# dpryan79/MethylDackel

Hardware: AMD Instinct MI355X
Metric: CpG calls/sec, synthetic 1 Mb contig 30x paired-end WGBS BAM, CpG extract (higher is better)
Workload: dtype u8/u32

## Files before the change

### include/mdk_hip.h

```cpp
#ifndef MDK_HIP_H
#define MDK_HIP_H
#include <stdint.h>
#ifdef __cplusplus
extern "C" {
#endif

#define MDK_ERR_HIP      (-1)
#define MDK_ERR_NODEVICE (-2)
#define MDK_ERR_ARG      (-3)
#define MDK_ERR_NOREF    (-4)
#define MDK_ERR_STRAND0  (-5)
#define MDK_ERR_NOMEM    (-6)
#define MDK_ERR_PREP_HOST (-7)

typedef struct md_dev md_dev;

typedef struct {
    int32_t keepCpG, keepCHG, keepCHH;
    int32_t minPhred;
    int32_t minOppositeDepth;
    int32_t bounds[16];
    int32_t absoluteBounds[16];
    int32_t tile;
    int32_t n_slots;
// ... 99 lines not shown
    float ms_pileup;
    uint64_t algo_bytes;
    uint64_t n_sites;
    int32_t tile, n_tiles, lds_bytes;
} md_bench_result;

int  md_dev_count(void);
int  md_dev_warm(int device);
void md_dev_quiesce(void);
void md_dev_reserve_hint(uint64_t device_bytes);
int  md_dev_open(int device, const md_dev_cfg *cfg, md_dev **out);
int  md_dev_reserve_contigs(md_dev *h, int32_t n);
void md_dev_close(md_dev *h);
const char *md_dev_last_error(void);
int  md_dev_tile(const md_dev *h);

int  md_dev_set_reference(md_dev *h, int32_t tid, const char *seq, int64_t len);

typedef struct { int32_t start, end, strand; } md_region;
int  md_dev_set_regions(md_dev *h, int32_t tid, const md_region *runs, int64_t n);

typedef struct { int32_t len; const uint32_t *count; } md_mbias;
int  md_dev_mbias_submit(md_dev *h, int slot, const md_read_batch *b);
int  md_dev_mbias_submit_raw(md_dev *h, int slot, const md_raw_batch *b);
int  md_dev_mbias_read(md_dev *h, md_mbias *out);
int  md_dev_mbias_reset(md_dev *h);
int  md_dev_slot_sync(md_dev *h, int slot);
int  md_dev_mbias_group(md_dev *h, const int *slots, int n);
int  md_dev_mbias_collect(md_dev *h, const int *slots, int n, int *rc);
int  md_dev_mbias_redone(const md_dev *h);
// ... 172 lines not shown
```

### methyldackel_amd/__init__.py

```python
from __future__ import annotations

import ctypes as C
import os
import struct
import subprocess
from pathlib import Path

ROOT = Path(__file__).resolve().parent
REPO = ROOT.parent
BUILD = Path(os.environ["MDK_BUILD_DIR"]) if os.environ.get("MDK_BUILD_DIR") else ROOT / "_build"
LIB_HIP = BUILD / "libmdk_hip.so"
LIB_EXTRACT = BUILD / "libmdk_extract.so"
CLI = BUILD / "MethylDackel"

CHUNK_NOREF, CHUNK_FOREIGN, CHUNK_BED = 1, 2, 4
CHUNK_EMPTY = CHUNK_NOREF | CHUNK_BED
MDK_ERR = {-1: "HIP call failed", -2: "no device", -3: "bad argument", -4: "reference not uploaded",
           -5: "strand 0 read reached a call", -6: "out of memory"}


class MdkError(RuntimeError):
    pass


# ... 116 lines not shown
    tables = any(bool(raw.range[i].h_rec_off) or bool(raw.range[i].d_rec_off) for i in range(raw.n_ranges))
    if not tables:
        return [raw.rec_off[i] for i in range(raw.n_records)]
    for i in range(raw.n_ranges):
        r = raw.range[i]
        if r.d_rec_off:
            raise MdkError("raw_record_offsets: a range lies in device memory")
        if r.h_rec_off:
            out += [r.h_rec_off[k] - r.rec_delta + o for k in range(r.n_records)]
        else:
            out += [raw.rec_off[hidx + k] for k in range(r.n_records)]; hidx += r.n_records
        o += r.bytes
    return out


HIP_SYMBOLS = ["md_dev_count", "md_dev_warm", "md_dev_quiesce", "md_dev_reserve_hint", "md_dev_open", "md_dev_close", "md_dev_last_error", "md_dev_tile", "md_dev_set_reference", "md_dev_set_regions",
               "md_dev_upload", "md_dev_launch", "md_dev_submit", "md_dev_download", "md_dev_sync", "md_dev_bind_output", "md_dev_wait", "md_sites_order",
               "md_dev_bench", "md_dev_bench_rotate", "md_dev_launch_group", "md_dev_group_max", "md_dev_download_group", "md_dev_reserve_contigs", "md_comm_unique_id", "md_comm_open_rank", "md_comm_open_rank_shared", "md_comm_close", "md_comm_world", "md_comm_gather", "md_comm_wait", "md_comm_result_header", "md_comm_result_send", "md_comm_result_recv", "md_dev_pci_bus_id",
               "md_bench_open", "md_bench_run", "md_bench_verify", "md_bench_region_bytes", "md_bench_close", "md_dev_debug_effective", "md_host_alloc", "md_host_free", "md_host_set_pinned", "md_host_profile", "md_dev_profile_text", "md_host_register", "md_host_register_all",
               "md_dev_set_prep", "md_dev_set_mappability", "md_dev_upload_raw", "md_dev_upload_raw_inplace", "md_dev_upload_wait", "md_dev_upload_done", "md_dev_submit_raw", "md_dev_debug_segments", "md_dev_bench_prep", "md_dev_bench_prep_rotate", "md_bench_set_prep",
               "md_dev_mbias_submit", "md_dev_mbias_submit_raw", "md_dev_mbias_read", "md_dev_mbias_reset", "md_dev_slot_sync",
               "md_dev_mbias_group", "md_dev_mbias_collect", "md_dev_mbias_redone", "md_dev_bias_finish", "md_bias_set_count", "md_bias_set_len", "md_bias_set_redone", "md_bias_set_hist", "md_bias_set_copy", "md_bias_set_free",
               "md_dev_perread_submit", "md_dev_perread_download", "md_dev_perread_submit_raw", "md_dev_perread_download_raw", "md_dev_read_raw",
               "md_piece_members_per_round", "md_piece_create", "md_piece_destroy", "md_piece_submit", "md_piece_wait", "md_piece_read", "md_piece_read_records", "md_piece_copy", "md_piece_bench", "md_piece_bench_crc",
               "md_dev_calls_begin", "md_dev_calls_group", "md_dev_calls_finish", "md_calls_set_count", "md_calls_set_copy", "md_calls_set_free", "md_dev_reset",
               "md_dev_reads_begin", "md_dev_reads_slot", "md_dev_reads_collect", "md_dev_reads_host", "md_dev_reads_finish", "md_reads_set_count", "md_reads_set_name_bytes", "md_reads_set_copy", "md_reads_set_free",
               "md_dev_cytosines_begin", "md_dev_cytosines_group", "md_dev_cytosines_finish", "md_cytosines_set_count", "md_cytosines_set_copy", "md_cytosines_set_free",
               "md_text_open", "md_text_measure_calls", "md_text_measure_cytosines", "md_text_measure_reads", "md_text_fill", "md_text_gather_names", "md_text_close", "md_text_merge_measure", "md_text_merge_fill", "md_text_regions", "md_text_unite_measure", "md_text_unite_fill", "md_text_diff", "md_text_dmr_measure", "md_text_dmr_fill",
               "md_text_reference", "md_text_parse_measure", "md_text_parse_fill_calls", "md_text_parse_fill_cytosines", "md_text_parse_error_offset", "md_text_deflate_measure", "md_text_deflate_fill"]
EXTRACT_SYMBOLS = ["extract_main", "mdk_plan_open", "mdk_plan_close", "mdk_plan_dev_cfg", "mdk_plan_ensure_reference",
                   "mdk_plan_next_chunk", "mdk_plan_try_next_chunk", "mdk_plan_emit", "mdk_plan_finish", "mdk_plan_set_shard", "mdk_plan_n_targets", "mdk_plan_target_name",
# ... 17 lines not shown
        print(r.stdout[-4000:], r.stderr[-4000:])
    if r.returncode:
        raise MdkError("build failed")


def lib_hip():
    global _hip
    if _hip is None:
        if not LIB_HIP.exists():
            raise MdkError(f"{LIB_HIP} is missing: the HIP extension was not built (run `make` / __graft_entry__.build()); there is no fallback")
        L = C.CDLL(str(LIB_HIP), mode=C.RTLD_GLOBAL)
        L.md_dev_last_error.restype = C.c_char_p
        L.md_dev_open.argtypes = [C.c_int, C.POINTER(md_dev_cfg), C.POINTER(C.c_void_p)]
        L.md_dev_close.argtypes = [C.c_void_p]
        L.md_dev_tile.argtypes = [C.c_void_p]
        L.md_dev_set_reference.argtypes = [C.c_void_p, C.c_int32, C.c_char_p, C.c_int64]
        L.md_dev_set_regions.argtypes = [C.c_void_p, C.c_int32, C.POINTER(md_region), C.c_int64]
        for f in ("md_dev_upload", "md_dev_submit"):
            getattr(L, f).argtypes = [C.c_void_p, C.c_int, C.POINTER(md_read_batch)]
        L.md_dev_launch.argtypes = [C.c_void_p, C.c_int]
        L.md_dev_download.argtypes = [C.c_void_p, C.c_int, C.POINTER(md_sites)]
        L.md_dev_sync.argtypes = [C.c_void_p]
        L.md_dev_bind_output.argtypes = [C.c_void_p, C.c_int, C.c_void_p, C.c_void_p, C.c_void_p, C.c_int64, C.c_int64]
        L.md_dev_wait.argtypes = [C.c_void_p, C.c_int, C.POINTER(md_sites_dev)]
        L.md_sites_order.argtypes = [C.c_void_p, C.c_void_p, C.c_void_p, C.c_int32, C.c_int64, C.c_void_p, C.c_void_p]
        L.md_sites_order.restype = C.c_int64
        L.md_dev_bench.argtypes = [C.c_void_p, C.c_int, C.c_int, C.c_int, C.POINTER(md_bench_result)]
        L.md_dev_bench_rotate.argtypes = [C.c_void_p, C.POINTER(C.c_int), C.c_int, C.c_int, C.c_int, C.c_int, C.POINTER(md_bench_result)]
        L.md_dev_launch_group.argtypes = [C.c_void_p, C.POINTER(C.c_int), C.c_int]
        L.md_comm_unique_id.argtypes = [C.c_char_p]
# ... 1723 lines not shown
```

### methyldackel_amd/csrc/mdk_hip.hip

```cpp
#include <sys/mman.h>
#include <atomic>
#include <mutex>
#include <algorithm>
#include <type_traits>
#include <condition_variable>
#include <thread>
#include <chrono>
#include "mdk_hip_internal.hpp"

#define DEFAULT_TILE 2048
#define PERMAX 4
#define MAX_TILE (WG * PERMAX)
#define LDS_LIMIT 163840

static thread_local char g_err[MDK_ERR_BYTES] = "";
char *mdk_err_buf() { return g_err; }
int fail(int code, const char *what, hipError_t e) {
    snprintf(g_err, sizeof(g_err), "%s: %s", what, e == hipSuccess ? "invalid argument" : hipGetErrorString(e));
    return code;
}

static std::atomic<uint64_t> g_prof_ns[PF_N], g_prof_calls[PF_N];
bool mdk_prof_on() { static const bool on = getenv("MDK_HOST_PROFILE") != nullptr; return on; }
double mdk_now() { return std::chrono::duration<double>(std::chrono::steady_clock::now().time_since_epoch()).count(); }
// ... 122 lines not shown
    p = harena_take(256); if(p) harena_give(p);
}


struct KParams {
    const md_seg *seg; const uint8_t *blob;
    const uint8_t *ctxcode; int64_t reflen;
    int64_t beg, end; int tile, ntiles, nper;
    const TileEnt *tiles;
    md_site *site; md_site_var *var; md_tile_seg *tseg; uint32_t *total, *total_next; int64_t cap_sites;
    int keepmask, minPhred;
    int bounds[16], abounds[16];
    int *err;
    int packed;
    int mbias; uint32_t *hist; int hist_lq;
};

__device__ __forceinline__ void trim_window(const KParams &P, int strand, int read2, int lq, int &lo, int &hi) {
    if(strand < 1) { lo = 0; hi = lq; return; }
    int b = 4 * (strand - 1) + (read2 ? 2 : 0);
    int lb = P.bounds[b], rb = P.bounds[b + 1];
    int alb = P.abounds[b], arb = P.abounds[b + 1];
    lb = lb < lq ? lb : lq; alb = alb < lq ? alb : lq; arb = arb < lq ? arb : lq;
    lo = lb > alb ? lb : alb;
    hi = (rb && rb < lq) ? rb : lq;
    if(lq - arb < hi) hi = lq - arb;
}

struct RD {
    int lq, lo, hi;
    const uint8_t *seq, *qual;
};
__device__ __forceinline__ RD make_rd(const KParams &P, uint32_t off4, uint32_t lq, int strand, int read2) {
    RD d; d.lq = (int)lq;
    if(P.packed) { d.seq = P.blob + off4; d.qual = d.seq + ((d.lq + 1) >> 1); }
    else { d.seq = P.blob + 4ull * off4; d.qual = d.seq + ((((d.lq + 1) >> 1) + 3) & ~3); }
    trim_window(P, strand, read2, d.lq, d.lo, d.hi);
    return d;
}

#include "mdk_overlap_rule.h"

__global__ __launch_bounds__(WG) void k_classify(const char *ref, uint8_t *code, int64_t n) {
    for(int64_t p = (int64_t)blockIdx.x * WG + threadIdx.x; p < n; p += (int64_t)gridDim.x * WG) {
        char c = ref[p] & 0x5f; int type, isG, out = 0;
        if(c == 'C') {
            isG = 0;
            if(p + 1 < n && (ref[p + 1] & 0x5f) == 'G') type = 0;
            else if(p + 2 < n && (ref[p + 2] & 0x5f) == 'G') type = 1;
            else type = 2;
            out = 1 + 2 * type + isG;
        } else if(c == 'G') {
// ... 10 lines not shown
__global__ __launch_bounds__(WG) void k_mask_regions(uint8_t *code, int64_t n, const md_region *runs, int64_t nruns) {
    for(int64_t p = (int64_t)blockIdx.x * WG + threadIdx.x; p < n; p += (int64_t)gridDim.x * WG) {
        const int c = code[p] & 15;
        if(!c) { code[p] = 0; continue; }
        int64_t a = 0, b = nruns;
        while(a < b) { const int64_t m = (a + b) >> 1; if((int64_t)runs[m].end <= p) a = m + 1; else b = m; }
        code[p] = (a < nruns && (int64_t)runs[a].start <= p) ? (uint8_t)(c | ((runs[a].strand & 3) << 4)) : (uint8_t)0;
    }
}

#define KB 2

template <bool VARIANT>
__device__ __forceinline__ void lane_seg(const KParams &P, const md_seg &g, int T0, int T1,
                                         const uint16_t *listC, int nC, const uint16_t *listG, int nG,
                                         uint32_t *cm, uint32_t *cu, uint32_t *co, uint32_t *cv) {
    const int send = g.rpos + (int)g.len;
    if(g.rpos >= T1 || send <= T0) return;
    const int strand = g.sf & MDK_SF_STRAND;
    const bool odd = strand & 1, second = (g.sf & MDK_SF_SECOND) != 0, partner = (g.sf & MDK_SF_PARTNER) != 0;
    const RD o = make_rd(P, g.off4, g.l_qseq, strand, g.sf & MDK_SF_READ2);
    RD m = o;
    if(partner) m = make_rd(P, g.m_off4, g.m_l_qseq, g.msf & MDK_SF_STRAND, g.msf & MDK_SF_READ2);
    const int lo_off = g.rpos > T0 ? g.rpos - T0 : 0, hi_off = (send < T1 ? send : T1) - T0;
    const int badrs = strand == 0 ? 6 : (odd ? 4 : 2);
#pragma unroll
    for(int pass = 0; pass < (VARIANT ? 2 : 1); pass++) {
        const bool callpass = pass == 0;
        const bool useC = (odd == callpass);
        const uint16_t *list = useC ? listC : listG; const int n = useC ? nC : nG;
        int a = 0, b = n;
        while(a < b) { int mid = (a + b) >> 1; if((int)(list[mid] & 0x1fff) < lo_off) a = mid + 1; else b = mid; }
        int i = a;
        while(i < n) {
            int li[KB];
#pragma unroll
            for(int k = 0; k < KB; k++) {
                li[k] = -1;
                if(i < n) { const int e = list[i], l = e & 0x1fff; if(l < hi_off) { li[k] = ((badrs >> (e >> 13)) & 1) ? -2 : l; i++; } else i = n; }
            }
            if(li[0] == -1) break;
            uint32_t sb[KB], qb[KB], msb[KB], mqb[KB];
#pragma unroll
            for(int k = 0; k < KB; k++) {
                sb[k] = 0xff; qb[k] = 0; msb[k] = 0xff; mqb[k] = 0;
                if(li[k] >= 0) {
                    const int d = T0 + li[k] - g.rpos, q = (int)g.q0 + d, mq = (int)g.m_q0 + d;
                    if(q >= o.lo && q < o.hi) { sb[k] = o.seq[q >> 1]; qb[k] = o.qual[q]; }
                    if(partner && mq >= m.lo && mq < m.hi) { msb[k] = m.seq[mq >> 1]; mqb[k] = m.qual[mq]; }
                }
            }
#pragma unroll
            for(int k = 0; k < KB; k++) {
                if(li[k] < 0) continue;
                const int d = T0 + li[k] - g.rpos, q = (int)g.q0 + d, mq = (int)g.m_q0 + d;
                int bq = (q & 1) ? (sb[k] & 15) : (sb[k] >> 4), ql = (int)qb[k];
                if(partner) { int mb = (mq & 1) ? (msb[k] & 15) : (msb[k] >> 4); ql = resolve_overlap(second, bq, ql, mb, (int)mqb[k]); }
                if(callpass) {
                    if(strand == 0) atomicExch(P.err, 1);
                    if(ql >= P.minPhred) {
                        if(odd) { if(bq == 2) atomicAdd(&cm[li[k]], 1u); else if(bq == 8) atomicAdd(&cu[li[k]], 1u); }
                        else { if(bq == 4) atomicAdd(&cm[li[k]], 1u); else if(bq == 1) atomicAdd(&cu[li[k]], 1u); }
                    }
                } else if(VARIANT) {
                    if(ql >= P.minPhred) {
                        atomicAdd(&co[li[k]], 1u);
// ... 185 lines not shown
    lds_barrier();
    int pre = incl - packed, tot = 0;
    for(int w = 0; w < WAVES; w++) { const int c = wsum[w]; if(w < wave) pre += c; tot += c; }
    nC = tot & 0xffff; nG = tot >> 16;
    int oc = pre & 0xffff, og = pre >> 16;
#pragma unroll
    for(int j = 0; j < PERMAX; j++) {
        if(j < PER && code[j]) {
            const uint16_t ent = (uint16_t)((tid * PER + j) | ((code[j] >> 4) << 13));
            if((code[j] - 1) & 1) listG[og++] = ent; else listC[oc++] = ent;
        }
    }
    lds_barrier();
}

template <bool VARIANT, bool QW>
__device__ __forceinline__ void pileup_tile(const KParams &P, const int t, const int b) {
    extern __shared__ __align__(16) uint32_t lds[];
    const int TILE = P.tile, PER = TILE / WG;
    uint32_t *cm = lds, *cu = lds + TILE, *co = lds + 2 * TILE, *cv = lds + 3 * TILE;
    uint16_t *listC = (uint16_t *)(lds + (VARIANT ? 4 : 2) * TILE), *listG = listC + TILE;
    __shared__ int wsum[WAVES];
    __shared__ uint32_t sbase;

    const int64_t T0 = P.beg + (int64_t)t * TILE;
    const int64_t T1 = (T0 + TILE < P.end) ? T0 + TILE : P.end;
    const int tlen = (int)(T1 - T0);
    const int tid = threadIdx.x, lane = tid & 63, wave = tid >> 6;
    if(t == 0 && tid == 0) *P.total_next = 0;

    const TileEnt te = P.tiles[t];
    const int first = te.last > te.first ? te.first : 0, last = te.last > te.first ? te.last : 0;
    int code[PERMAX];
    load_codes(P, T0, tlen, PER, tid, code);
    md_seg g0; g0.rpos = 0x7fffffff; g0.len = 0;
    if(first + tid < last) g0 = P.seg[first + tid];

#pragma unroll
    for(int j = 0; j < PERMAX; j++) {
        if(j < PER) {
            const int i = tid * PER + j;
            cm[i] = 0; cu[i] = 0;
            if(VARIANT) { co[i] = 0; cv[i] = 0; }
        }
    }
    int nC, nG;
    build_lists(P, PER, tid, lane, wave, code, listC, listG, wsum, nC, nG);

    uint32_t codes = 0;
#pragma unroll
    for(int j = 0; j < PERMAX; j++) codes |= (uint32_t)(code[j] & 0xff) << (8 * j);
    asm volatile("" : "+v"(codes));

    if constexpr(QW) {
        const int topC = nC ? 1 << (31 - __clz(nC)) : 0, topG = nG ? 1 << (31 - __clz(nG)) : 0;
        for(int r0 = first; r0 < last; r0 += WG) {
            md_seg g = g0;
            if(r0 != first) { g.rpos = 0x7fffffff; g.len = 0; if(r0 + tid < last) g = P.seg[r0 + tid]; }
#ifndef QW_NO_SORT
            const SegQ sq = seg_sort(seg_setup<VARIANT>(P, g, (int)T0, (int)T1, listC, nC, nG, topC, topG), lane);
#else
            const SegQ sq = seg_setup<VARIANT>(P, g, (int)T0, (int)T1, listC, nC, nG, topC, topG);
#endif
            quarter_sites<VARIANT>(P, sq, lane, listC, cm, cu, co, cv);
        }
    } else {
        if(first + tid < last) lane_seg<VARIANT>(P, g0, (int)T0, (int)T1, listC, nC, listG, nG, cm, cu, co, cv);
        for(int r = first + WG + tid; r < last; r += WG) {
            const md_seg g = P.seg[r];
            lane_seg<VARIANT>(P, g, (int)T0, (int)T1, listC, nC, listG, nG, cm, cu, co, cv);
        }
    }
    uint32_t reserved = 0;
    if(tid == 0) reserved = (nC + nG) ? atomicAdd(P.total, (uint32_t)(nC + nG)) : 0u;
    __syncthreads();

#pragma unroll
    for(int j = 0; j < PERMAX; j++) code[j] = (int)((codes >> (8 * j)) & 0xffu);
    uint32_t vm[PERMAX], vu[PERMAX], vo[PERMAX], vv[PERMAX]; int cnt = 0;
#pragma unroll
    for(int j = 0; j < PERMAX; j++) {
        vm[j] = vu[j] = vo[j] = vv[j] = 0;
        const int i = tid * PER + j;
        if(j < PER && i < tlen && code[j]) { vm[j] = cm[i]; vu[j] = cu[i]; if(VARIANT) { vo[j] = co[i]; vv[j] = cv[i]; } }
        if((vm[j] + vu[j]) > 0 || vo[j] > 0) cnt++;
    }
    const int incl = wave_scan_incl(cnt, lane);
    if(lane == 63) wsum[wave] = incl;
    if(tid == 0) sbase = reserved;
    __syncthreads();
    if(tid == 0) {
        int tot = 0; for(int w = 0; w < WAVES; w++) tot += wsum[w];
        md_tile_seg sg; sg.off = reserved; sg.cnt = (uint32_t)tot; P.tseg[t] = sg;
    }
    {
        uint32_t o = sbase + (uint32_t)(incl - cnt);
        for(int w = 0; w < wave; w++) o += (uint32_t)wsum[w];
#pragma unroll
        for(int j = 0; j < PERMAX; j++) {
            if((vm[j] + vu[j]) > 0 || vo[j] > 0) {
                if((int64_t)o < P.cap_sites) {
                    md_site rec; rec.pos = (uint32_t)(T0 + tid * PER + j); rec.nmeth = vm[j]; rec.nunmeth = vu[j]; rec.meta = (uint32_t)((code[j] & 15) - 1);
                    P.site[o] = rec;
                    if(VARIANT) { md_site_var rv; rv.noff = vo[j]; rv.nvar = vv[j]; P.var[o] = rv; }
                }
                o++;
            }
        }
// ... 315 lines not shown
    if(side_streams) { std::unique_lock<std::mutex> lk(g_stash_mu); g_stash_cv.wait_for(lk, std::chrono::milliseconds(500), [] { return g_warm_streams_made.load() >= WARM_STREAMS; }); }
    else for(int i = 0; i < WARM_STREAMS; i++) {
        hipStream_t s = nullptr;
        if(hipStreamCreateWithFlags(&s, hipStreamNonBlocking) != hipSuccess) { (void)hipGetLastError(); break; }
        { std::lock_guard<std::mutex> lk(g_stash_mu);
          if(g_stash_dev != device) { g_stash.clear(); g_stash_dev = device; }
          g_stash.push_back(s); }
        g_stash_cv.notify_all();
    }
    const double t4 = mdk_now();
    arena_prime(device);
    if(mdk_prof_on()) fprintf(stderr, "[mdk hip] warm-up: runtime init + device count %.3fs, context (hipSetDevice + hipFree(0)) %.3fs, the library's code object %.3fs, %d streams %.3fs, first blocks of carved device / pinned memory %.3fs\n", t1 - t0, t2 - t1, t3 - t2, WARM_STREAMS, t4 - t3, mdk_now() - t4);
    return 0;
}

static int fixed_lds(int tile, bool variant) { return tile * ((variant ? 16 : 8) + 4); }

extern "C" int md_dev_open(int device, const md_dev_cfg *cfg, md_dev **out) {
    if(!cfg || !out) return fail(MDK_ERR_ARG, "md_dev_open", hipSuccess);
    *out = nullptr;
    const double t_open0 = mdk_now();
    for(int q = 0; q < 256; q++) {
        uint8_t v = (uint8_t)q; v = (uint8_t)(int)(v + 0.2 * v);
        if(v != (uint8_t)(((q * 6) / 5) & 255)) { snprintf(g_err, sizeof(g_err), "boost identity fails at q=%d", q); return MDK_ERR_ARG; }
    }
    int n = md_dev_count();
    if(n <= 0) { if(n == 0) snprintf(g_err, sizeof(g_err), "no HIP device visible"); return MDK_ERR_NODEVICE; }
    if(device < 0 || device >= n) return fail(MDK_ERR_ARG, "md_dev_open: device index", hipSuccess);
    HIPCHK(hipSetDevice(device));
    g_warm_reg_stop.store(true);
    if(code_object_load()) return fail(MDK_ERR_HIP, "loading the device library's code object", hipGetLastError());
    md_dev *h = new md_dev();
    h->device = device; h->cfg = *cfg;
    h->tile = cfg->tile > 0 ? cfg->tile : ((cfg->keepCHG || cfg->keepCHH) ? 1536 : DEFAULT_TILE);
    h->tile = (h->tile + WG - 1) / WG * WG;
    if(h->tile > MAX_TILE) h->tile = MAX_TILE;
    h->n_slots = cfg->n_slots > 0 ? cfg->n_slots : 2;
    h->variant = cfg->minOppositeDepth > 0;
    h->qw = (cfg->keepCHG || cfg->keepCHH) && !getenv("MDK_NO_QW");
    while(fixed_lds(h->tile, h->variant) > LDS_LIMIT - 1024 && h->tile > WG) h->tile -= WG;
    if(fixed_lds(h->tile, h->variant) > 65536) {
        HIPCHK(hipFuncSetAttribute(pileup_fn(h->variant, h->qw), hipFuncAttributeMaxDynamicSharedMemorySize, fixed_lds(h->tile, h->variant)));
        HIPCHK(hipFuncSetAttribute(pileup_multi_fn(h->variant, h->qw), hipFuncAttributeMaxDynamicSharedMemorySize, fixed_lds(h->tile, h->variant)));
    }
    h->slots.resize(h->n_slots);
    if(h->d_status.need((size_t)h->n_slots) || h->h_status.need((size_t)h->n_slots)) return MDK_ERR_NOMEM;
    HIPCHK(hipMemset(h->d_status.p, 0, sizeof(SlotStatus) * (size_t)h->n_slots));
    HIPCHK(hipDeviceSynchronize());
    memset(h->h_status.p, 0, sizeof(SlotStatus) * (size_t)h->n_slots);
    for(int i = 0; i < h->n_slots; i++) { Slot &s = h->slots[i]; s.index = i; s.d_total.p = h->d_status.p[i].total; s.d_err.p = &h->d_status.p[i].err; s.d_pcnt.p = &h->d_status.p[i].pc; s.h_st.p = &h->h_status.p[i]; }
    const double t_open1 = mdk_now();
    const bool shared = cfg->n_streams > 0;
    const int n_streams = shared ? std::min(cfg->n_streams, (h->n_slots + MAXM - 1) / MAXM) : h->n_slots;
    for(int i = 0; i < n_streams; i++) { hipStream_t st = stream_take(device); if(!st) return fail(MDK_ERR_HIP, "hipStreamCreateWithFlags", hipGetLastError()); h->streams.push_back(st); }
    for(auto &s : h->slots) {
        s.stream = h->streams[(size_t)(shared ? s.index / MAXM : s.index) % (size_t)n_streams];
        HIPCHK(hipEventCreate(&s.e0)); HIPCHK(hipEventCreate(&s.e1)); HIPCHK(hipEventCreate(&s.k0)); HIPCHK(hipEventCreate(&s.k1));
        s.run = s.stream;
    }
// ... 62 lines not shown
    for(Slot &s : h->slots) {
        slot_buffers_release(s);
        Slot f;
        f.stream = s.stream; f.e0 = s.e0; f.e1 = s.e1; f.k0 = s.k0; f.k1 = s.k1; f.index = s.index; f.run = s.stream; f.ring = s.ring;
        s = f;
    }
    h->d_status.release(); h->h_status.release();
    mdk_debug_state("md_dev_reset, released");
    arena_restart_if_idle(h->device); harena_restart_if_idle();
    if(h->d_status.need((size_t)h->n_slots) || h->h_status.need((size_t)h->n_slots)) return MDK_ERR_NOMEM;
    HIPCHK(hipMemset(h->d_status.p, 0, sizeof(SlotStatus) * (size_t)h->n_slots));
    HIPCHK(hipDeviceSynchronize());
    memset(h->h_status.p, 0, sizeof(SlotStatus) * (size_t)h->n_slots);
    for(Slot &s : h->slots) { s.d_total.p = h->d_status.p[s.index].total; s.d_err.p = &h->d_status.p[s.index].err; s.d_pcnt.p = &h->d_status.p[s.index].pc; s.h_st.p = &h->h_status.p[s.index]; }
    h->cfg = *cfg;
    h->tile = cfg->tile > 0 ? cfg->tile : ((cfg->keepCHG || cfg->keepCHH) ? 1536 : DEFAULT_TILE);
    h->tile = (h->tile + WG - 1) / WG * WG;
    if(h->tile > MAX_TILE) h->tile = MAX_TILE;
    h->variant = cfg->minOppositeDepth > 0;
    h->qw = (cfg->keepCHG || cfg->keepCHH) && !getenv("MDK_NO_QW");
    while(fixed_lds(h->tile, h->variant) > LDS_LIMIT - 1024 && h->tile > WG) h->tile -= WG;
    if(fixed_lds(h->tile, h->variant) > 65536) {
        HIPCHK(hipFuncSetAttribute(pileup_fn(h->variant, h->qw), hipFuncAttributeMaxDynamicSharedMemorySize, fixed_lds(h->tile, h->variant)));
        HIPCHK(hipFuncSetAttribute(pileup_multi_fn(h->variant, h->qw), hipFuncAttributeMaxDynamicSharedMemorySize, fixed_lds(h->tile, h->variant)));
    }
    return 0;
}

extern "C" int md_dev_tile(const md_dev *h) { return h ? h->tile : MDK_ERR_ARG; }

extern "C" int md_dev_reserve_contigs(md_dev *h, int32_t n) {
    if(!h || n < 0) return fail(MDK_ERR_ARG, "md_dev_reserve_contigs", hipSuccess);
    const size_t k = (size_t)n;
    if(h->ref.size() < k) { h->ref.resize(k, nullptr); h->refcode.resize(k, nullptr); h->reflen.resize(k, 0); }
    if(h->ref_carved.size() < k) h->ref_carved.resize(k, 0);
    if(h->d_runs.size() < k) { h->d_runs.resize(k, nullptr); h->n_runs.resize(k, 0); h->has_runs.resize(k, 0); }
    if(h->mapbits.size() < k) { h->mapbits.resize(k, nullptr); h->maplen.resize(k, 0); }
    return 0;
}

static void ref_release(md_dev *h, size_t tid) {
// ... 76 lines not shown
    if(b->tid < 0 || (size_t)b->tid >= h->ref.size() || !h->ref[b->tid]) { snprintf(g_err, sizeof(g_err), "reference for tid %d not uploaded", b->tid); return MDK_ERR_NOREF; }
    HIPCHK(hipSetDevice(h->device));
    if(s->busy) {
        HIPCHK(hipStreamSynchronize(s->stream));
        if(s->run && s->run != s->stream) HIPCHK(hipStreamSynchronize(s->run));
    }
    s->busy = true;
    s->fresh = true;
    if((uint64_t)b->blob_bytes >= (1ull << 32) - 64) return fail(MDK_ERR_ARG, "md_dev_upload: more than 4 GiB of read payload in one chunk", hipSuccess);
    const int64_t span = b->end - b->beg;
    s->n_segs = b->n_segs; s->n_reads = b->n_reads; s->tid = b->tid; s->beg = b->beg; s->end = b->end; s->uploaded = false; s->launched = false; s->raw_layout = false;
    const int TILE = h->tile;
    const int ntiles = (int)((span + TILE - 1) / TILE);
    if(s->h_tiles.need((size_t)(ntiles > 0 ? ntiles : 1))) return MDK_ERR_NOMEM;
    build_tiles(b, TILE, s->h_tiles.p, ntiles);
    s->tile = TILE; s->ntiles = ntiles; s->lds_bytes = fixed_lds(TILE, h->variant);
    s->read_bytes = b->algo_bytes;
    size_t ns = (size_t)b->n_segs, nt = (size_t)(ntiles > 0 ? ntiles : 1);
    if(s->d_seg_in.need(ns + 1) || s->d_blob.need((size_t)b->blob_bytes + 64)) return MDK_ERR_NOMEM;
    if(s->d_tiles.need(nt) || s->d_seg.need(nt)) return MDK_ERR_NOMEM;
    if(!s->b_site) {
        if(s->d_site.need((size_t)span + 16)) return MDK_ERR_NOMEM;
        if(h->variant && s->d_var.need((size_t)span + 16)) return MDK_ERR_NOMEM;
    }
    if(ns) {
        host_block_ensure_registered(b->seg); host_block_ensure_registered(b->blob);
        HIPCHK(hipMemcpyAsync(s->d_seg_in.p, b->seg, ns * sizeof(md_seg), hipMemcpyHostToDevice, s->stream));
        HIPCHK(hipMemcpyAsync(s->d_blob.p, b->blob, (size_t)b->blob_bytes, hipMemcpyHostToDevice, s->stream));
    }
    if(ntiles) HIPCHK(hipMemcpyAsync(s->d_tiles.p, s->h_tiles.p, nt * sizeof(TileEnt), hipMemcpyHostToDevice, s->stream));
    s->uploaded = true;
// ... 12 lines not shown
static int fill_kparams(md_dev *h, Slot *s, KParams &P) {
    memset(&P, 0, sizeof(P));
    P.seg = s->d_seg_in.p; P.blob = s->raw_layout ? const_cast<uint8_t *>(s->raw_at) : s->d_blob.p; P.packed = s->raw_layout ? 1 : 0;
    P.ctxcode = h->refcode[s->tid]; P.reflen = h->reflen[s->tid];
    P.beg = s->beg; P.end = s->end; P.tile = s->tile; P.ntiles = s->ntiles; P.nper = (s->ntiles + 7) / 8;
    P.tiles = s->d_tiles.p;
    if(s->b_site) {
        if(s->b_cap_tiles < s->ntiles) return fail(MDK_ERR_ARG, "bound tile-segment buffer too small", hipSuccess);
        P.site = s->b_site; P.var = s->b_var; P.tseg = s->b_seg; P.cap_sites = s->b_cap_sites;
    } else { P.site = s->d_site.p; P.var = s->d_var.p; P.tseg = s->d_seg.p; P.cap_sites = (int64_t)s->d_site.cap; }
    P.total = s->d_total.p + (s->ring % RING); P.total_next = s->d_total.p + ((s->ring + 1) % RING);
    P.keepmask = (h->cfg.keepCpG ? 1 : 0) | (h->cfg.keepCHG ? 2 : 0) | (h->cfg.keepCHH ? 4 : 0);
    P.minPhred = h->cfg.minPhred;
    for(int i = 0; i < 16; i++) { P.bounds[i] = h->cfg.bounds[i]; P.abounds[i] = h->cfg.absoluteBounds[i]; }
    P.err = s->d_err.p;
    return 0;
}

int launch_kernels(md_dev *h, Slot *s, bool time_pileup, hipStream_t on) {
    hipStream_t st = on ? on : s->stream;
    if(s->fresh && st != s->stream) { HIPCHK(hipEventRecord(s->e0, s->stream)); HIPCHK(hipStreamWaitEvent(st, s->e0, 0)); }
    if(s->raw_layout && s->prep_pending) { Slot *one[1] = {s}; int rc = enqueue_prep_group(h, one, 1, st); if(rc) return rc; }
    s->fresh = false; s->run = st; s->packed = false;
    s->ring++;
    if(s->ntiles > 0) {
        KParams P; int rc = fill_kparams(h, s, P); if(rc) return rc;
        int grid = P.nper * 8;
        if(time_pileup) HIPCHK(hipEventRecord(s->k0, st));
        launch_pileup(h, grid, (size_t)s->lds_bytes, st, P);
        if(time_pileup) HIPCHK(hipEventRecord(s->k1, st));
// ... 688 lines not shown
```

### methyldackel_amd/csrc/mdk_hip_internal.hpp

```cpp
#ifndef MDK_HIP_INTERNAL_HPP
#define MDK_HIP_INTERNAL_HPP
#include <hip/hip_runtime.h>
#include <stdint.h>
#include <stdio.h>
#include <stdlib.h>
#include <string.h>
#include <atomic>
#include <vector>
#include <mutex>
#include "mdk_hip.h"

#ifndef WG
#define WG 512
#endif
#define WAVES (WG / 64)
#define RING 64
#define MAXM 8

#define MDK_HIDDEN __attribute__((visibility("hidden")))
MDK_HIDDEN char *mdk_err_buf();
#define MDK_ERR_BYTES 512
MDK_HIDDEN int fail(int code, const char *what, hipError_t e);
#define HIPCHK(call) do { hipError_t e_ = (call); if(e_ != hipSuccess) return fail(MDK_ERR_HIP, #call, e_); } while(0)

MDK_HIDDEN int mdk_mark_begin(const char *what);
// ... 73 lines not shown
    int n_segs = 0, n_reads = 0, ntiles = 0, tid = -1, tile = 0, lds_bytes = 0; int64_t beg = 0, end = 0; uint64_t read_bytes = 0;
    bool uploaded = false, launched = false; unsigned ring = 0;
    double t_launch = 0;
    bool packed = false;
    bool busy = false;
};

struct CallsState;
MDK_HIDDEN void calls_state_free(md_dev *h);
struct ReadsState;
MDK_HIDDEN void reads_state_free(md_dev *h);
struct CytoState;
MDK_HIDDEN void cyto_state_free(md_dev *h);
struct md_dev {
    int device; md_dev_cfg cfg; int tile, n_slots; bool variant; bool qw = false;
    CallsState *calls = nullptr; bool no_pack = false;
    ReadsState *reads = nullptr; bool reads_on = false;
    CytoState *cyto = nullptr;
    std::vector<hipStream_t> streams;
    std::mutex crc_mu; void *d_crc = nullptr;
    std::mutex piece_mu; std::vector<hipStream_t> piece_streams; int piece_rr = 0; hipStream_t piece_in = nullptr, piece_inf = nullptr;
    hipStream_t ref_stream = nullptr;
    std::vector<Slot> slots;
    std::vector<char *> ref; std::vector<uint8_t *> refcode; std::vector<int64_t> reflen; std::vector<char> ref_carved; std::vector<int64_t> refcap;
    DBuf<SlotStatus> d_status; HBuf<SlotStatus> h_status;
    md_prep_cfg prep; bool prep_set = false; std::vector<uint32_t *> mapbits; std::vector<int64_t> maplen;
    std::vector<md_region *> d_runs; std::vector<int64_t> n_runs; std::vector<char> has_runs;
    uint32_t *d_hist = nullptr; int hist_cap = 0, hist_len = 0; std::vector<uint32_t> h_hist;
    std::mutex mb_mu; int mb_redone = 0, mb_hint = 0;
    std::atomic<bool> scan_wide{getenv("MDK_SCAN_WIDE") && atoi(getenv("MDK_SCAN_WIDE")) > 0}; bool scan_wide_fixed = getenv("MDK_SCAN_WIDE") != nullptr;
// ... 47 lines not shown
    if(lane == 63) wtot[wave] = x;
    __syncthreads();
    T before = 0; total = 0;
    for(int w = 0; w < WGS / 64; w++) { const T t = wtot[w]; if(w < wave) before += t; total += t; }
    __syncthreads();
    return before + x - v;
}

enum { PF_UP_SYNC = 0, PF_UP_ALLOC, PF_UP_COPY, PF_LAUNCH, PF_FIN_WAIT, PF_DL_COPY, PF_DL_ORDER, PF_SETREF, PF_PIECE_SUBMIT, PF_PIECE_WAIT, PF_GRP_DEV, PF_GRP_TURN, PF_N };
MDK_HIDDEN bool mdk_prof_on();
MDK_HIDDEN void mdk_prof_add(int site, double seconds);
MDK_HIDDEN double mdk_now();
struct ProfScope { int site; double t0; ProfScope(int s) : site(s), t0(mdk_prof_on() ? mdk_now() : 0.0) {} ~ProfScope() { if(mdk_prof_on()) mdk_prof_add(site, mdk_now() - t0); } };
MDK_HIDDEN Slot *get_slot(md_dev *h, int slot);
MDK_HIDDEN void host_block_ensure_registered(const void *ptr);
MDK_HIDDEN int launch_kernels(md_dev *h, Slot *s, bool time_pileup, hipStream_t on = nullptr);
MDK_HIDDEN int launch_group_on(md_dev *h, const int *slots, int n, hipStream_t on, bool cross_sync);
MDK_HIDDEN int64_t finish_count(md_dev *h, Slot *s);
MDK_HIDDEN int64_t finish_eval(md_dev *h, Slot *s);
MDK_HIDDEN int finish_group(md_dev *h, const int *slots, int n, int64_t *counts);
MDK_HIDDEN int prep_outcome(md_dev *h, Slot *s);
MDK_HIDDEN int prep_kernels_init();
MDK_HIDDEN void inflate_kernels_warm();
MDK_HIDDEN hipStream_t mdk_piece_stream_take(int device);
MDK_HIDDEN hipStream_t mdk_stream_take(int device);
MDK_HIDDEN void mdk_debug_state(const char *where);
MDK_HIDDEN int mbias_drain(md_dev *h);
MDK_HIDDEN int enqueue_prep_group(md_dev *h, Slot *const *ss, int n, hipStream_t st);
struct ColSpec { uint32_t elem, extra; };
#define COLTAB_MAXK 8
// ... 52 lines not shown
```

### methyldackel_amd/csrc/mdk_prep.hip

```cpp
#include <algorithm>
#include <atomic>
#include <mutex>
#include "mdk_hip_internal.hpp"
#include "mdk_pair_rule.h"

#ifndef PB
#define PB 256
#endif
#define MAXG 16
#define CNT_READY 0x80000000u

__device__ __forceinline__ uint32_t ld16(const uint8_t *p) { uint16_t v; __builtin_memcpy(&v, p, 2); return v; }
__device__ __forceinline__ uint32_t ld32(const uint8_t *p) { uint32_t v; __builtin_memcpy(&v, p, 4); return v; }
__device__ __forceinline__ uint64_t ld64(const uint8_t *p) { uint64_t v; __builtin_memcpy(&v, p, 8); return v; }
__device__ __forceinline__ uint4 ld128(const uint8_t *p) { uint4 v; __builtin_memcpy(&v, p, 16); return v; }

struct PrepParams {
    const uint8_t *raw; uint64_t raw_bytes; const uint32_t *rec_off; int n_rec;
    md_prep_cfg cfg; int32_t tid; int64_t beg, end, woff, wlen;
    const char *ref; int64_t reflen;
    const uint32_t *mapbits; int64_t maplen;
    const md_region *runs; int64_t nruns; int bed_on;
    PrepRead *rd; uint32_t *aidx;
    unsigned long long *hent; int32_t *hnext, *hfwd; uint32_t hmask;
// ... 1015 lines not shown
        ~SlowCall() { if(on) { const double t = mdk_now(); if(t - t0 > 0.004) { char w[256]; snprintf(w, sizeof(w), "slow upload_raw: %.1f ms (slot wait %.1f, buffers %.1f, copies %.1f), %d ranges, %d records, first range %s", (t - t0) * 1e3, (t_sync - t0) * 1e3, (t_alloc - t_sync) * 1e3, (t - t_alloc) * 1e3, b->n_ranges, b->n_records, b->n_ranges ? (b->range[0].d_rec_off ? "device" : b->range[0].h_rec_off ? "host+table" : "host") : "-"); mdk_marks_dump(w); } } } } slow(b);
    if(s->busy) {
        ProfScope pf(PF_UP_SYNC);
        HIPCHK(hipStreamSynchronize(s->stream));
        if(s->run && s->run != s->stream) HIPCHK(hipStreamSynchronize(s->run));
    }
    slow.t_sync = slow.on ? mdk_now() : 0;
    s->busy = true;
    s->fresh = true;
    uint64_t total = 0;
    for(int i = 0; i < b->n_ranges; i++) total += b->range[i].bytes;
    if(total >= (1ull << 32) - 64) return fail(MDK_ERR_ARG, "md_dev_upload_raw: more than 4 GiB of records in one chunk", hipSuccess);
    const int64_t span = b->end - b->beg; const int TILE = h->tile;
    const int ntiles = (int)((span + TILE - 1) / TILE), n = b->n_records, nb = (n + PB - 1) / PB;
    s->tid = b->tid; s->beg = b->beg; s->end = b->end; s->woff = b->woff; s->wlen = b->wlen; s->uploaded = false; s->launched = false;
    s->tile = TILE; s->ntiles = ntiles; s->lds_bytes = TILE * ((h->variant ? 16 : 8) + 4);
    s->pr_nrec = n; s->raw_bytes = total; s->raw_layout = true; s->n_segs = -1; s->n_reads = -1; s->read_bytes = 0;
    static const bool no_inplace = getenv("MDK_NO_INPLACE") != nullptr;
    const bool inplace = may_stay && !no_inplace && b->n_ranges == 1 && b->range[0].d_rec_off && (uint32_t)n == b->range[0].n_records && n > 0 && b->range[0].bytes + (uint64_t)b->range[0].rec_delta < (1ull << 32) - 64;
    const size_t nn = (size_t)n + 1, nt = (size_t)(ntiles > 0 ? ntiles : 1);
    const size_t segcap = std::max<size_t>(s->d_seg_in.cap, nn * 2 + 4096);
    s->hmask = pow2_at_least(nn + nn / 4) - 1;
    static std::atomic<int> first_call{1}; const bool first = mdk_prof_on() && first_call.exchange(0); const double tf0 = first ? mdk_now() : 0; double tf1 = 0;
    {
        ProfScope pf(PF_UP_ALLOC);
        if((!inplace && (s->d_raw.need((size_t)total + 64) || s->d_recoff.need(nn))) || s->d_prd.need(nn) || s->d_hnext.need(2 * nn + 8) || s->d_zero.need(zero_bytes_for(s->hmask, nb)) ||
           s->d_seg_in.need(segcap) || s->d_tiles.need(nt) || s->d_seg.need(nt)) return MDK_ERR_NOMEM;
        if(!s->b_site) {
            if(s->d_site.need((size_t)span + 16)) return MDK_ERR_NOMEM;
            if(h->variant && s->d_var.need((size_t)span + 16)) return MDK_ERR_NOMEM;
        }
// ... 151 lines not shown
```

Before: 6.866 billion.

## Prefetch pileup segments into LDS with async global_load_lds double buffering

Adds per-wave LDS staging windows, sized to fit in LDS left over without lowering workgroups per CU. Each wave prefetches the next batch of 32-byte segment records into LDS with inline global_load_lds_dwordx4 while it processes the current batch. This hides global latency in the segment loop. The trim bounds move into an LDS table, and the atomic output reservation moves earlier onto a thread in the last wave so it overlaps the segment work. Risks include fragile inline asm with manual m0 and waitcnt handling, and extra LDS per block.

```diff
diff --git a/include/mdk_hip.h b/include/mdk_hip.h
--- a/include/mdk_hip.h
+++ b/include/mdk_hip.h
@@ -137,6 +137,7 @@
 void md_dev_close(md_dev *h);
 const char *md_dev_last_error(void);
 int  md_dev_tile(const md_dev *h);
+int  md_dev_stage_segments(md_dev *h);
 
 int  md_dev_set_reference(md_dev *h, int32_t tid, const char *seq, int64_t len);
 
diff --git a/methyldackel_amd/__init__.py b/methyldackel_amd/__init__.py
--- a/methyldackel_amd/__init__.py
+++ b/methyldackel_amd/__init__.py
@@ -154,7 +154,7 @@
     return out
 
 
-HIP_SYMBOLS = ["md_dev_count", "md_dev_warm", "md_dev_quiesce", "md_dev_reserve_hint", "md_dev_open", "md_dev_close", "md_dev_last_error", "md_dev_tile", "md_dev_set_reference", "md_dev_set_regions",
+HIP_SYMBOLS = ["md_dev_count", "md_dev_warm", "md_dev_quiesce", "md_dev_reserve_hint", "md_dev_open", "md_dev_close", "md_dev_last_error", "md_dev_tile", "md_dev_stage_segments", "md_dev_set_reference", "md_dev_set_regions",
                "md_dev_upload", "md_dev_launch", "md_dev_submit", "md_dev_download", "md_dev_sync", "md_dev_bind_output", "md_dev_wait", "md_sites_order",
                "md_dev_bench", "md_dev_bench_rotate", "md_dev_launch_group", "md_dev_group_max", "md_dev_download_group", "md_dev_reserve_contigs", "md_comm_unique_id", "md_comm_open_rank", "md_comm_open_rank_shared", "md_comm_close", "md_comm_world", "md_comm_gather", "md_comm_wait", "md_comm_result_header", "md_comm_result_send", "md_comm_result_recv", "md_dev_pci_bus_id",
                "md_bench_open", "md_bench_run", "md_bench_verify", "md_bench_region_bytes", "md_bench_close", "md_dev_debug_effective", "md_host_alloc", "md_host_free", "md_host_set_pinned", "md_host_profile", "md_dev_profile_text", "md_host_register", "md_host_register_all",
@@ -202,6 +202,7 @@
         L.md_dev_open.argtypes = [C.c_int, C.POINTER(md_dev_cfg), C.POINTER(C.c_void_p)]
         L.md_dev_close.argtypes = [C.c_void_p]
         L.md_dev_tile.argtypes = [C.c_void_p]
+        L.md_dev_stage_segments.argtypes = [C.c_void_p]
         L.md_dev_set_reference.argtypes = [C.c_void_p, C.c_int32, C.c_char_p, C.c_int64]
         L.md_dev_set_regions.argtypes = [C.c_void_p, C.c_int32, C.POINTER(md_region), C.c_int64]
         for f in ("md_dev_upload", "md_dev_submit"):
diff --git a/methyldackel_amd/csrc/mdk_hip.hip b/methyldackel_amd/csrc/mdk_hip.hip
--- a/methyldackel_amd/csrc/mdk_hip.hip
+++ b/methyldackel_amd/csrc/mdk_hip.hip
@@ -160,13 +160,16 @@
     int *err;
     int packed;
     int mbias; uint32_t *hist; int hist_lq;
+    int stage_waves;
 };
 
-__device__ __forceinline__ void trim_window(const KParams &P, int strand, int read2, int lq, int &lo, int &hi) {
+template <bool TB = false>
+__device__ __forceinline__ void trim_window(const KParams &P, int strand, int read2, int lq, int &lo, int &hi, const int *tb = nullptr) {
     if(strand < 1) { lo = 0; hi = lq; return; }
     int b = 4 * (strand - 1) + (read2 ? 2 : 0);
-    int lb = P.bounds[b], rb = P.bounds[b + 1];
-    int alb = P.abounds[b], arb = P.abounds[b + 1];
+    int lb, rb, alb, arb;
+    if constexpr(TB) { lb = tb[b]; rb = tb[b + 1]; alb = tb[16 + b]; arb = tb[16 + b + 1]; }
+    else { lb = P.bounds[b]; rb = P.bounds[b + 1]; alb = P.abounds[b]; arb = P.abounds[b + 1]; }
     lb = lb < lq ? lb : lq; alb = alb < lq ? alb : lq; arb = arb < lq ? arb : lq;
     lo = lb > alb ? lb : alb;
     hi = (rb && rb < lq) ? rb : lq;
@@ -177,11 +180,12 @@
     int lq, lo, hi;
     const uint8_t *seq, *qual;
 };
-__device__ __forceinline__ RD make_rd(const KParams &P, uint32_t off4, uint32_t lq, int strand, int read2) {
+template <bool TB = false>
+__device__ __forceinline__ RD make_rd(const KParams &P, uint32_t off4, uint32_t lq, int strand, int read2, const int *tb = nullptr) {
     RD d; d.lq = (int)lq;
     if(P.packed) { d.seq = P.blob + off4; d.qual = d.seq + ((d.lq + 1) >> 1); }
     else { d.seq = P.blob + 4ull * off4; d.qual = d.seq + ((((d.lq + 1) >> 1) + 3) & ~3); }
-    trim_window(P, strand, read2, d.lq, d.lo, d.hi);
+    trim_window<TB>(P, strand, read2, d.lq, d.lo, d.hi, tb);
     return d;
 }
 
@@ -222,14 +226,14 @@
 template <bool VARIANT>
 __device__ __forceinline__ void lane_seg(const KParams &P, const md_seg &g, int T0, int T1,
                                          const uint16_t *listC, int nC, const uint16_t *listG, int nG,
-                                         uint32_t *cm, uint32_t *cu, uint32_t *co, uint32_t *cv) {
+                                         uint32_t *cm, uint32_t *cu, uint32_t *co, uint32_t *cv, const int *tb) {
     const int send = g.rpos + (int)g.len;
     if(g.rpos >= T1 || send <= T0) return;
     const int strand = g.sf & MDK_SF_STRAND;
     const bool odd = strand & 1, second = (g.sf & MDK_SF_SECOND) != 0, partner = (g.sf & MDK_SF_PARTNER) != 0;
-    const RD o = make_rd(P, g.off4, g.l_qseq, strand, g.sf & MDK_SF_READ2);
+    const RD o = make_rd<true>(P, g.off4, g.l_qseq, strand, g.sf & MDK_SF_READ2, tb);
     RD m = o;
-    if(partner) m = make_rd(P, g.m_off4, g.m_l_qseq, g.msf & MDK_SF_STRAND, g.msf & MDK_SF_READ2);
+    if(partner) m = make_rd<true>(P, g.m_off4, g.m_l_qseq, g.msf & MDK_SF_STRAND, g.msf & MDK_SF_READ2, tb);
     const int lo_off = g.rpos > T0 ? g.rpos - T0 : 0, hi_off = (send < T1 ? send : T1) - T0;
     const int badrs = strand == 0 ? 6 : (odd ? 4 : 2);
 #pragma unroll
@@ -258,6 +262,8 @@
                     if(partner && mq >= m.lo && mq < m.hi) { msb[k] = m.seq[mq >> 1]; mqb[k] = m.qual[mq]; }
                 }
             }
+#pragma unroll
+            for(int k = 0; k < KB; k++) asm volatile("" :: "v"(sb[k]), "v"(qb[k]), "v"(msb[k]), "v"(mqb[k]));
 #pragma unroll
             for(int k = 0; k < KB; k++) {
                 if(li[k] < 0) continue;
@@ -473,6 +479,20 @@
     lds_barrier();
 }
 
+#define RSV_TID (WG - 64)
+
+__device__ __forceinline__ void stage_segs(const md_seg *seg, const int base, const int last, int tid, const uint32_t win) {
+    asm volatile("" : "+v"(tid));
+#pragma unroll
+    for(int k = 0; k < 2; k++) {
+        const int p = 64 * k + (tid & 63), s = base + (p >> 1);
+        if(s < last) {
+            const uint8_t *src = (const uint8_t *)(seg + s) + 16 * (p & 1); uint32_t keep;
+            asm volatile("s_mov_b32 %0, m0\n\ts_mov_b32 m0, %2\n\ts_nop 0\n\tglobal_load_lds_dwordx4 %1, off\n\ts_mov_b32 m0, %0" : "=&s"(keep) : "v"(src), "s"(__builtin_amdgcn_readfirstlane(win + 1024u * k)) : "memory");
+        }
+    }
+}
+
 template <bool VARIANT, bool QW>
 __device__ __forceinline__ void pileup_tile(const KParams &P, const int t, const int b) {
     extern __shared__ __align__(16) uint32_t lds[];
@@ -481,6 +501,7 @@
     uint16_t *listC = (uint16_t *)(lds + (VARIANT ? 4 : 2) * TILE), *listG = listC + TILE;
     __shared__ int wsum[WAVES];
     __shared__ uint32_t sbase;
+    __shared__ int tbl[32];
 
     const int64_t T0 = P.beg + (int64_t)t * TILE;
     const int64_t T1 = (T0 + TILE < P.end) ? T0 + TILE : P.end;
@@ -494,6 +515,17 @@
     load_codes(P, T0, tlen, PER, tid, code);
     md_seg g0; g0.rpos = 0x7fffffff; g0.len = 0;
     if(first + tid < last) g0 = P.seg[first + tid];
+    const int *const tb = tbl;
+    if(!QW && wave == WAVES - 1) {
+        int v = 0;
+#pragma unroll
+        for(int i = 0; i < 16; i++) { if(lane == i) v = P.bounds[i]; if(lane == 16 + i) v = P.abounds[i]; }
+        if(lane < 32) tbl[lane] = v;
+    }
+    const int uwave = __builtin_amdgcn_readfirstlane(wave);
+    const uint32_t win = (uint32_t)(uintptr_t)(__attribute__((address_space(3))) uint8_t *)((uint8_t *)(listC + 2 * TILE) + MDK_STAGE_WAVE_BYTES * uwave);
+    const bool staged = !QW && uwave < P.stage_waves;
+    if(staged) stage_segs(P.seg, first + WG + 64 * uwave, last, tid, win);
 
 #pragma unroll
     for(int j = 0; j < PERMAX; j++) {
@@ -505,6 +537,8 @@
     }
     int nC, nG;
     build_lists(P, PER, tid, lane, wave, code, listC, listG, wsum, nC, nG);
+
+    if(tid == RSV_TID) sbase = (nC + nG) ? atomicAdd(P.total, (uint32_t)(nC + nG)) : 0u;
 
     uint32_t codes = 0;
 #pragma unroll
@@ -524,14 +558,27 @@
             quarter_sites<VARIANT>(P, sq, lane, listC, cm, cu, co, cv);
         }
     } else {
-        if(first + tid < last) lane_seg<VARIANT>(P, g0, (int)T0, (int)T1, listC, nC, listG, nG, cm, cu, co, cv);
-        for(int r = first + WG + tid; r < last; r += WG) {
-            const md_seg g = P.seg[r];
-            lane_seg<VARIANT>(P, g, (int)T0, (int)T1, listC, nC, listG, nG, cm, cu, co, cv);
-        }
-    }
-    uint32_t reserved = 0;
-    if(tid == 0) reserved = (nC + nG) ? atomicAdd(P.total, (uint32_t)(nC + nG)) : 0u;
+        if(first + tid < last) lane_seg<VARIANT>(P, g0, (int)T0, (int)T1, listC, nC, listG, nG, cm, cu, co, cv, tb);
+        if(staged) {
+            for(int rb = first + WG + 64 * uwave; rb < last; rb += WG) {
+                asm volatile("s_waitcnt vmcnt(0)" ::: "memory");
+                __builtin_amdgcn_wave_barrier();
+                int l = tid; asm volatile("" : "+v"(l)); l &= 63;
+                const uint4 *const rec = (const uint4 *)((__attribute__((address_space(3))) uint8_t *)(uintptr_t)win + 32 * l);
+                uint4 w0 = rec[0], w1 = rec[1];
+                asm volatile("s_waitcnt lgkmcnt(0)" : "+v"(w0.x), "+v"(w0.y), "+v"(w0.z), "+v"(w0.w), "+v"(w1.x), "+v"(w1.y), "+v"(w1.z), "+v"(w1.w) :: "memory");
+                __builtin_amdgcn_wave_barrier();
+                stage_segs(P.seg, rb + WG, last, tid, win);
+                md_seg g; __builtin_memcpy(&g, &w0, 16); __builtin_memcpy((char *)&g + 16, &w1, 16);
+                if(rb + l < last) lane_seg<VARIANT>(P, g, (int)T0, (int)T1, listC, nC, listG, nG, cm, cu, co, cv, tb);
+            }
+        } else {
+            for(int r = first + WG + tid; r < last; r += WG) {
+                const md_seg g = P.seg[r];
+                lane_seg<VARIANT>(P, g, (int)T0, (int)T1, listC, nC, listG, nG, cm, cu, co, cv, tb);
+            }
+        }
+    }
     __syncthreads();
 
 #pragma unroll
@@ -546,11 +593,10 @@
     }
     const int incl = wave_scan_incl(cnt, lane);
     if(lane == 63) wsum[wave] = incl;
-    if(tid == 0) sbase = reserved;
     __syncthreads();
-    if(tid == 0) {
+    if(tid == RSV_TID) {
         int tot = 0; for(int w = 0; w < WAVES; w++) tot += wsum[w];
-        md_tile_seg sg; sg.off = reserved; sg.cnt = (uint32_t)tot; P.tseg[t] = sg;
+        md_tile_seg sg; sg.off = sbase; sg.cnt = (uint32_t)tot; P.tseg[t] = sg;
     }
     {
         uint32_t o = sbase + (uint32_t)(incl - cnt);
@@ -896,7 +942,23 @@
     return 0;
 }
 
-static int fixed_lds(int tile, bool variant) { return tile * ((variant ? 16 : 8) + 4); }
+static int stage_waves_of(int tile, bool variant, bool qw) { return pileup_stage_waves(tile, variant, !qw, qw ? QW_WAVES : PILEUP_WAVES, WAVES); }
+int pileup_lds_of(const md_dev *h) { return pileup_fixed_lds(h->tile, h->variant) + MDK_STAGE_WAVE_BYTES * h->stage_waves; }
+static int set_geometry(md_dev *h, const md_dev_cfg *cfg) {
+    h->tile = cfg->tile > 0 ? cfg->tile : ((cfg->keepCHG || cfg->keepCHH) ? 1536 : DEFAULT_TILE);
+    h->tile = (h->tile + WG - 1) / WG * WG;
+    if(h->tile > MAX_TILE) h->tile = MAX_TILE;
+    h->variant = cfg->minOppositeDepth > 0;
+    h->qw = (cfg->keepCHG || cfg->keepCHH) && !getenv("MDK_NO_QW");
+    while(pileup_fixed_lds(h->tile, h->variant) > LDS_LIMIT - 1024 && h->tile > WG) h->tile -= WG;
+    h->stage_waves = stage_waves_of(h->tile, h->variant, h->qw);
+    if(pileup_lds_of(h) > 65536) {
+        HIPCHK(hipFuncSetAttribute(pileup_fn(h->variant, h->qw), hipFuncAttributeMaxDynamicSharedMemorySize, pileup_lds_of(h)));
+        HIPCHK(hipFuncSetAttribute(pileup_multi_fn(h->variant, h->qw), hipFuncAttributeMaxDynamicSharedMemorySize, pileup_lds_of(h)));
+    }
+    return 0;
+}
+extern "C" int md_dev_stage_segments(md_dev *h) { return h ? 64 * h->stage_waves : MDK_ERR_ARG; }
 
 extern "C" int md_dev_open(int device, const md_dev_cfg *cfg, md_dev **out) {
     if(!cfg || !out) return fail(MDK_ERR_ARG, "md_dev_open", hipSuccess);
@@ -914,17 +976,8 @@
     if(code_object_load()) return fail(MDK_ERR_HIP, "loading the device library's code object", hipGetLastError());
     md_dev *h = new md_dev();
     h->device = device; h->cfg = *cfg;
-    h->tile = cfg->tile > 0 ? cfg->tile : ((cfg->keepCHG || cfg->keepCHH) ? 1536 : DEFAULT_TILE);
-    h->tile = (h->tile + WG - 1) / WG * WG;
-    if(h->tile > MAX_TILE) h->tile = MAX_TILE;
     h->n_slots = cfg->n_slots > 0 ? cfg->n_slots : 2;
-    h->variant = cfg->minOppositeDepth > 0;
-    h->qw = (cfg->keepCHG || cfg->keepCHH) && !getenv("MDK_NO_QW");
-    while(fixed_lds(h->tile, h->variant) > LDS_LIMIT - 1024 && h->tile > WG) h->tile -= WG;
-    if(fixed_lds(h->tile, h->variant) > 65536) {
-        HIPCHK(hipFuncSetAttribute(pileup_fn(h->variant, h->qw), hipFuncAttributeMaxDynamicSharedMemorySize, fixed_lds(h->tile, h->variant)));
-        HIPCHK(hipFuncSetAttribute(pileup_multi_fn(h->variant, h->qw), hipFuncAttributeMaxDynamicSharedMemorySize, fixed_lds(h->tile, h->variant)));
-    }
+    { const int rc = set_geometry(h, cfg); if(rc) { delete h; return rc; } }
     h->slots.resize(h->n_slots);
     if(h->d_status.need((size_t)h->n_slots) || h->h_status.need((size_t)h->n_slots)) return MDK_ERR_NOMEM;
     HIPCHK(hipMemset(h->d_status.p, 0, sizeof(SlotStatus) * (size_t)h->n_slots));
@@ -1017,17 +1070,7 @@
     memset(h->h_status.p, 0, sizeof(SlotStatus) * (size_t)h->n_slots);
     for(Slot &s : h->slots) { s.d_total.p = h->d_status.p[s.index].total; s.d_err.p = &h->d_status.p[s.index].err; s.d_pcnt.p = &h->d_status.p[s.index].pc; s.h_st.p = &h->h_status.p[s.index]; }
     h->cfg = *cfg;
-    h->tile = cfg->tile > 0 ? cfg->tile : ((cfg->keepCHG || cfg->keepCHH) ? 1536 : DEFAULT_TILE);
-    h->tile = (h->tile + WG - 1) / WG * WG;
-    if(h->tile > MAX_TILE) h->tile = MAX_TILE;
-    h->variant = cfg->minOppositeDepth > 0;
-    h->qw = (cfg->keepCHG || cfg->keepCHH) && !getenv("MDK_NO_QW");
-    while(fixed_lds(h->tile, h->variant) > LDS_LIMIT - 1024 && h->tile > WG) h->tile -= WG;
-    if(fixed_lds(h->tile, h->variant) > 65536) {
-        HIPCHK(hipFuncSetAttribute(pileup_fn(h->variant, h->qw), hipFuncAttributeMaxDynamicSharedMemorySize, fixed_lds(h->tile, h->variant)));
-        HIPCHK(hipFuncSetAttribute(pileup_multi_fn(h->variant, h->qw), hipFuncAttributeMaxDynamicSharedMemorySize, fixed_lds(h->tile, h->variant)));
-    }
-    return 0;
+    return set_geometry(h, cfg);
 }
 
 extern "C" int md_dev_tile(const md_dev *h) { return h ? h->tile : MDK_ERR_ARG; }
@@ -1134,7 +1177,7 @@
     const int ntiles = (int)((span + TILE - 1) / TILE);
     if(s->h_tiles.need((size_t)(ntiles > 0 ? ntiles : 1))) return MDK_ERR_NOMEM;
     build_tiles(b, TILE, s->h_tiles.p, ntiles);
-    s->tile = TILE; s->ntiles = ntiles; s->lds_bytes = fixed_lds(TILE, h->variant);
+    s->tile = TILE; s->ntiles = ntiles; s->lds_bytes = pileup_lds_of(h);
     s->read_bytes = b->algo_bytes;
     size_t ns = (size_t)b->n_segs, nt = (size_t)(ntiles > 0 ? ntiles : 1);
     if(s->d_seg_in.need(ns + 1) || s->d_blob.need((size_t)b->blob_bytes + 64)) return MDK_ERR_NOMEM;
@@ -1177,6 +1220,7 @@
     P.minPhred = h->cfg.minPhred;
     for(int i = 0; i < 16; i++) { P.bounds[i] = h->cfg.bounds[i]; P.abounds[i] = h->cfg.absoluteBounds[i]; }
     P.err = s->d_err.p;
+    P.stage_waves = h->stage_waves;
     return 0;
 }
 
diff --git a/methyldackel_amd/csrc/mdk_hip_internal.hpp b/methyldackel_amd/csrc/mdk_hip_internal.hpp
--- a/methyldackel_amd/csrc/mdk_hip_internal.hpp
+++ b/methyldackel_amd/csrc/mdk_hip_internal.hpp
@@ -9,6 +9,7 @@
 #include <vector>
 #include <mutex>
 #include "mdk_hip.h"
+#include "mdk_pileup_lds.h"
 
 #ifndef WG
 #define WG 512
@@ -112,6 +113,7 @@
 MDK_HIDDEN void cyto_state_free(md_dev *h);
 struct md_dev {
     int device; md_dev_cfg cfg; int tile, n_slots; bool variant; bool qw = false;
+    int stage_waves = 0;
     CallsState *calls = nullptr; bool no_pack = false;
     ReadsState *reads = nullptr; bool reads_on = false;
     CytoState *cyto = nullptr;
@@ -189,6 +191,7 @@
 struct ProfScope { int site; double t0; ProfScope(int s) : site(s), t0(mdk_prof_on() ? mdk_now() : 0.0) {} ~ProfScope() { if(mdk_prof_on()) mdk_prof_add(site, mdk_now() - t0); } };
 MDK_HIDDEN Slot *get_slot(md_dev *h, int slot);
 MDK_HIDDEN void host_block_ensure_registered(const void *ptr);
+MDK_HIDDEN int pileup_lds_of(const md_dev *h);
 MDK_HIDDEN int launch_kernels(md_dev *h, Slot *s, bool time_pileup, hipStream_t on = nullptr);
 MDK_HIDDEN int launch_group_on(md_dev *h, const int *slots, int n, hipStream_t on, bool cross_sync);
 MDK_HIDDEN int64_t finish_count(md_dev *h, Slot *s);
diff --git a/methyldackel_amd/csrc/mdk_pileup_lds.h b/methyldackel_amd/csrc/mdk_pileup_lds.h
--- /dev/null
+++ b/methyldackel_amd/csrc/mdk_pileup_lds.h
@@ -0,0 +1,26 @@
+#ifndef MDK_PILEUP_LDS_H
+#define MDK_PILEUP_LDS_H
+
+#define MDK_LDS_PER_CU 163840
+#define MDK_PILEUP_STATIC_LDS 176
+#define MDK_STAGE_WAVE_BYTES 2048
+
+static inline int pileup_fixed_lds(int tile, int variant) { return tile * ((variant ? 16 : 8) + 4); }
+
+static inline int pileup_wgs_per_cu(int dyn_bytes, int waves_per_simd, int wg_waves) {
+    const int by_waves = waves_per_simd * 4 / wg_waves, by_lds = MDK_LDS_PER_CU / (dyn_bytes + MDK_PILEUP_STATIC_LDS);
+    return by_waves < by_lds ? by_waves : by_lds;
+}
+
+static inline int pileup_stage_waves(int tile, int variant, int staged_form, int waves_per_simd, int wg_waves) {
+    if(!staged_form || tile <= 0) return 0;
+    const int fixed = pileup_fixed_lds(tile, variant), want = pileup_wgs_per_cu(fixed, waves_per_simd, wg_waves);
+    int n = wg_waves;
+    while(n > 0 && pileup_wgs_per_cu(fixed + n * MDK_STAGE_WAVE_BYTES, waves_per_simd, wg_waves) != want) n--;
+    return n;
+}
+
+static inline int pileup_lds_bytes(int tile, int variant, int staged_form, int waves_per_simd, int wg_waves) {
+    return pileup_fixed_lds(tile, variant) + MDK_STAGE_WAVE_BYTES * pileup_stage_waves(tile, variant, staged_form, waves_per_simd, wg_waves);
+}
+#endif
diff --git a/methyldackel_amd/csrc/mdk_prep.hip b/methyldackel_amd/csrc/mdk_prep.hip
--- a/methyldackel_amd/csrc/mdk_prep.hip
+++ b/methyldackel_amd/csrc/mdk_prep.hip
@@ -1053,7 +1053,7 @@
     const int64_t span = b->end - b->beg; const int TILE = h->tile;
     const int ntiles = (int)((span + TILE - 1) / TILE), n = b->n_records, nb = (n + PB - 1) / PB;
     s->tid = b->tid; s->beg = b->beg; s->end = b->end; s->woff = b->woff; s->wlen = b->wlen; s->uploaded = false; s->launched = false;
-    s->tile = TILE; s->ntiles = ntiles; s->lds_bytes = TILE * ((h->variant ? 16 : 8) + 4);
+    s->tile = TILE; s->ntiles = ntiles; s->lds_bytes = pileup_lds_of(h);
     s->pr_nrec = n; s->raw_bytes = total; s->raw_layout = true; s->n_segs = -1; s->n_reads = -1; s->read_bytes = 0;
     static const bool no_inplace = getenv("MDK_NO_INPLACE") != nullptr;
     const bool inplace = may_stay && !no_inplace && b->n_ranges == 1 && b->range[0].d_rec_off && (uint32_t)n == b->range[0].n_records && n > 0 && b->range[0].bytes + (uint64_t)b->range[0].rec_delta < (1ull << 32) - 64;
```

Measured after the change: 6.874 billion, median of 6. Within noise of the previous version (+0.1%).
